# marvinx97/cloud

Measured on AMD Instinct MI355X. Metric: images/sec ResNet-50 via run() at 1/2/4/8 MI355X; run()→first-step latency, higher is better.
Workload: dtype bf16

## Files before the change

### cloud_amd/config.py

```python
from __future__ import annotations

import os
from dataclasses import dataclass


@dataclass(frozen=True)
class Var:
    name: str
    type: type
    default: object
    doc: str
    area: str


_VARS = [
    Var("CLOUD_AMD_JOBS_DIR", str, "./jobs", "where run() stages job directories", "launcher"),
    Var("CLOUD_AMD_HOME", str, "~/.cloud_amd", "per-user state: the job-id index (jobs/<id> -> job directory) that "
        "python -m cloud_amd.jobs uses to find a job from any directory", "launcher"),
    Var("CLOUD_AMD_STAGE_COPY", bool, False, "stage code files by copying too (default: code "
        "hard-linked, every other file copied; a running job then never sees in-place edits of its sources)", "launcher"),
    Var("CLOUD_AMD_CPU_AFFINITY", bool, True, "launcher pins each GPU rank to the cores of its GPU's NUMA node "
        "(KFD io_links + sysfs cpulist), split between the ranks on that node; 0 = leave placement to the OS",
        "launcher"),
    Var("CLOUD_AMD_NUMA_ROOT", str, "/sys/devices/system/node", "sysfs NUMA-node tree read for rank CPU placement "
# ... 49 lines not shown
        "the workgroups (one contiguous sweep); 0 = one contiguous row chunk per workgroup", "ops"),
    Var("CLOUD_AMD_CONV_TALL", bool, True, "<= 64-channel 3x3 convolutions (fwd, stride-1 dgrad): 256 x 64 tiles "
        "with 4 x 1 waves; 0 = 128 x 64 with 2 x 2 waves", "ops"),
    Var("CLOUD_AMD_STEM_LDS", bool, True, "space-to-depth stem convolution forward on the LDS-resident patch + filter "
        "kernel (csrc/include/ca_conv_stem.h); 0 = the implicit-GEMM row-segment loader", "ops"),
    Var("CLOUD_AMD_STEM_TALL", bool, True, "space-to-depth stem convolution on the tall 256 x 64 tiles too (0.88 -> "
        "0.72 ms per call at b1024); 0 = 128 x 64 tiles (A/B runs)", "ops"),
    Var("CLOUD_AMD_STEM_BWD_RECOMPUTE", bool, True, "ResNet stem tail backward: a statistics-only max-pool "
        "backward pass, then the BN-backward apply recomputes the pooled gradient per 2x2 block (the 112x112 "
        "gradient is never written: 3.3 GB fewer per step at b1024).  With the window loads issued ahead of "
        "any branch: 0.65 + 0.90 ms against 1.09 + 0.94 for write-then-apply, +0.8 % end to end "
        "(profiles/r4_s44/); 0 = write g and run the separate apply pass", "ops"),
    Var("CLOUD_AMD_BN_GROUPS_MAX", int, 512, "BatchNorm statistics: most groups of the first-level reduction of the "
        "per-tile partial rows (1..512; ~64 rows per group)", "ops"),
    Var("CLOUD_AMD_GEMM_LIB", str, "never", "plain bf16 GEMMs (bias / accumulate only, no fused epilogue): 'never' "
        "(default: every GEMM on the in-tree kernels, the same engine on every box and rank), 'auto' (diagnostic: "
        "times the in-tree kernel against hipBLASLt once per shape and keeps the faster), 'always' "
        "(ops/raw.py PlainGemmPolicy)", "ops"),
    Var("CLOUD_AMD_GEMM_PRW", bool, True, "forward 1x1 convolutions with N = 256, K = 64 (ResNet layer-1 conv3 "
        "and shortcut): persistent resident-weight core (csrc/include/ca_gemm_prw.h); 0 = the tiled 128 core",
        "ops"),
    Var("CLOUD_AMD_GEMM_PRWN", bool, True, "forward 1x1 convolutions N = 512 / K = 128 and N = 1024 / K = 256 with "
        "BN statistics (ResNet stage-2 / stage-3 conv3): the persistent core with the weight resident in column "
        "chunks (ca_gemm_prw.h); 0 = the tiled 128 core", "ops"),
    Var("CLOUD_AMD_SMALLK_SET", str, "", "bench/smallk_gemm.py shape set ('conv3': the conv3 expansions of "
        "stages 2-4)", "bench"),
    Var("CLOUD_AMD_EPI_PF", bool, True, "GEMM epilogues that read memory or run an activation (BN-statistics "
        "and inference-BN forward 1x1 convs, BERT bias/GELU/GELU'/beta dense layers): 4 staged output rows in flight per trip", "ops"),
    Var("CLOUD_AMD_EPI_PIPE", bool, True, "input-gradient GEMMs / convolutions with the BN-backward statistics "
        "epilogue: the next two output rows' operand loads are in flight under this pair's arithmetic and stores "
        "(ca_mfma_core.h gemm_epilogue); 0 = one pair at a time (A/B runs)", "ops"),
    Var("CLOUD_AMD_ATTN_FUSED_BWD", bool, True,"attention at S = 64 / 128: one workgroup per (batch, head) for "
        "the forward and a single fused backward kernel; 0 keeps the 64-query-block kernels", "ops"),
    Var("CLOUD_AMD_CONV_HALO_WGRAD", bool, True, "the weight gradient of the same 3x3 / 64-channel / width-56 "
        "convolutions on the LDS-resident kernel (ca_conv_halo.h conv3x3_halo_wgrad: 64 x 576 partial in registers, "
        "one fp32 slab per workgroup); 0 = implicit GEMM (A/B)", "ops"),
    Var("CLOUD_AMD_LN_BWD16", bool, False, "LayerNorm backward on 16-wave blocks, one row per wave, the block's "
        "partials summed by a fixed LDS tree (measured 2.8 % slower on BERT beside the weight-gradient side stream; "
        "default: 4-wave blocks walking four rows per wave)", "ops"),
    Var("CLOUD_AMD_GEMM_256X96", bool, True, "forward GEMMs whose 256 x 96 grid fills whole rounds while the 128 x "
        "128 grid leaves a partial one (BERT QKV, M = 8192, N = 2304) run on 256 x 96 tiles; 0 = off (A/B)", "ops"),
    Var("CLOUD_AMD_BN_FIN_RPG", int, 512, "BatchNorm statistics finalize: partial rows per group block (64-512)", "ops"),
    Var("CLOUD_AMD_BN_FIN_MERGED", bool, True, "BatchNorm statistics from many partial rows: group reduction and "
        "per-channel finalize in ONE launch (last block per 64 channels finalizes, agent-scope ticket); 0 = two "
        "launches (A/B runs)", "ops"),
    Var("CLOUD_AMD_CONV_HALO", int, 1, "3x3 / stride-1 / 64-channel convolutions at width 56 (ResNet-50 "
        "stage 1) forward and input gradient on the LDS-resident kernel (ca_conv_halo.h: input patch and all 9 taps "
        "in LDS, persistent grid); 0 = implicit-GEMM tiles, 2 = halo kernel without the software-pipelined "
        "fragment reads (A/B runs)", "ops"),
    Var("CLOUD_AMD_CONV_PATCH", bool, True, "3x3 / stride-1 / pad-1 convolutions with a 64-multiple gathered channel "
        "count, more than 64 output columns and W <= 28 (ResNet-50 stages 2-4), forward and input gradient, on the "
        "patch-fed core (ca_conv_patch.h: the tile's input rows go to LDS once per 64-channel chunk, not once per "
        "tap); 0 = tap-gathered implicit GEMM (A/B runs)", "ops"),
    Var("CLOUD_AMD_CONV_EPI_PF", bool, True, "implicit-GEMM forward convolutions with the BN-statistics epilogue, and "
        "with the inference BN + residual + ReLU epilogue: read 2 staged output rows from LDS before storing", "ops"),
    Var("CLOUD_AMD_INFER_FUSE", bool, True, "ResNet blocks and stem that are not training (eval mode, or a frozen "
        "Keras base) under torch.no_grad(): every BatchNorm (+ residual + ReLU) in the epilogue of its convolution "
        "(ops.conv_bn_act_infer, ca_conv_fwd_bn) and no BN-statistics partials; 0 = the per-layer route "
        "(convolution with statistics, then bn_apply)", "ops"),
    Var("CLOUD_AMD_SHAPE_LOG", str, None, "profiling: append one JSON line per GEMM/convolution launch (kind, M, N, "
        "K, minimum HBM bytes) to this file, for scripts/gemm_roofline.py", "ops"),
    Var("CLOUD_AMD_BN_FOLD", bool, True, "ResNet block backward: the bn3 / bn1 backward apply runs in the operand "
        "fetch of the 1x1 input-gradient GEMM that consumes it (ca_gemm_xa.h) instead of a separate pass", "ops"),
    Var("CLOUD_AMD_BN_FOLD_FWD", bool, True, "ResNet block forward: bn2's apply runs in conv3's operand fetch and "
        "bn3's (+ residual) in the next block's conv1 (ca_gemm_xa.h); the applied tensors are written once, by "
        "those GEMMs", "ops"),
    Var("CLOUD_AMD_BN_FOLD_MAX_N", int, 256, "BN fold sites kept: only GEMMs with K >= 2N and N <= this "
        "(ResNet-50 default: bn3 -> conv3 dgrad and bn3 -> next conv1 at stages 1-3, the stage-3 ones on the two-deep "
        "128 x 256 transform-A tiles, CLOUD_AMD_XA_N256=3: +0.6 / +1.0 % on two boxes, docs/performance.md round 6; "
        "4096 = every stage); the short-K sites (bn2 -> conv3, bn1 -> conv1 dgrad) measured slower than the separate "
        "pass, and stage 4 (N 512) +0.3 % below stages 1-3 only", "ops"),
    Var("CLOUD_AMD_BN_FOLD_WGRAD", bool, True, "bn3 -> conv3 fold at 64 input channels (ResNet stage 1): conv3's weight "
        "gradient runs in the same kernel as its input gradient (ca_gemm_xa.h mfma_gemm_xa_dw), so the BN-backward "
        "output dz3 is never written", "ops"),
    Var("CLOUD_AMD_BN_FOLD_DS", bool, False, "ResNet projection blocks, stages 2-4: the shortcut BN's backward apply "
        "runs in the operand fetch of the sparse strided shortcut input-gradient GEMM (ca_gemm_xa_bwd_strided); A/B",
        "ops"),
    Var("CLOUD_AMD_DS_SPARSE_DGRAD", bool, True, "ResNet projection blocks with a strided 1x1 shortcut: the "
        "shortcut's input gradient is written for its one non-empty output-parity class only, and conv1's input "
        "gradient accumulates into it reading the other pixels as zeros -- no zero-fill of 3/4 of dx and no read "
        "of those zeros", "ops"),
    Var("CLOUD_AMD_BN_FOLD_WGRAD_DS", bool, True, "stage-1 projection shortcut: its BN backward (gated by the block "
        "output's ReLU mask), the shortcut conv's input gradient and its weight gradient in one pass", "ops"),
    Var("CLOUD_AMD_BN_FOLD_WGRAD2", bool, False, "the same one-pass input + weight gradient for stage 2's conv3 "
        "(K = 512 -> N = 128, 8-wave workgroups holding the 512 x 128 dW block)", "ops"),
    Var("CLOUD_AMD_BN_FOLD_WGRAD1", bool, False, "the same one-pass input + weight gradient for stage 1's conv1 with "
        "bn1's backward apply (K = 64 -> N = 256: dz1 never written, four output chunks per tile)", "ops"),
    Var("CLOUD_AMD_XA_N256", int, 3, "transform-A GEMMs (BN folded into a 1x1 conv) with N a multiple of 256: "
        "1 = 128 x 256 tiles on 16-wave workgroups (each A tile transformed once), "
        "3 (and any other value) = 16 waves with two K tiles' operands in flight (coefficients staged in LDS; K <= 2048), "
        "0 = 128 x 128 tiles.  Only the fold sites CLOUD_AMD_BN_FOLD_MAX_N admits reach them (ResNet-50 stage 3 "
        "at the default; measured in docs/performance.md, round 6)", "ops"),
    Var("CLOUD_AMD_XA_WAVES", int, 8,"128 x 128 transform-A GEMMs (BN folded into the 1x1 convs): 8-wave "
        "workgroups (<= 128 registers, two per CU) or 4", "ops"),
    Var("CLOUD_AMD_XA_WAVES_N64", bool, True, "the 128 x 64 transform-A GEMMs (stage 1) on 8-wave workgroups too "
        "(with CLOUD_AMD_XA_WAVES=8)", "ops"),
    Var("CLOUD_AMD_XA_DW_WAVES", int, 4, "stage-1 conv3 fused input+weight gradient: 4-wave workgroups (two per "
        "CU) or 8 (one per CU); 8 selects the one-step form", "ops"),
    Var("CLOUD_AMD_XA_DW_DEPTH", int, 1, "stage-1 fused input+weight gradient (K 256 -> N 64): 0 = one-step form; "
        "1, 2, 4 = deep form (weights resident in LDS, epilogue operands ahead of the next tile's) with that many "
        "source steps in flight per workgroup (1: two workgroups per CU, 2 and 4: one)", "ops"),
    Var("CLOUD_AMD_BN_FOLD_ALL", bool, False, "fold every BN site regardless of CLOUD_AMD_BN_FOLD_MAX_N (tests, A/B)",
        "ops"),
    Var("CLOUD_AMD_MAX_STEPS_IN_FLIGHT", int, 2, "training loops (benches, Keras fit) let the host enqueue at most this "
        "many steps ahead of the GPU (runtime.step_pacer); bounds the memory in flight so the caching allocator "
        "stops requesting segments after warmup; 0 = unbounded", "runtime"),
    Var("CLOUD_AMD_RUN_AHEAD_MS", float, 25.0, "the step pacer deepens its bound (up to 4 steps) so the queued steps "
# ... 143 lines not shown
```

### csrc/bindings.cpp

```cpp
#include <atomic>
#include <mutex>
#include <hip/hip_runtime.h>
#include <pybind11/pybind11.h>
#include <pybind11/stl.h>
#include <stdint.h>

#include <stdexcept>
#include <string>
#include <vector>

namespace py = pybind11;
typedef uint16_t bf16_t;

extern "C" {
int ca_sgd_step(float*, void*, int, float*, bf16_t*, const float*, const float*, long, int, int, hipStream_t);
int ca_adam_step(float*, void*, int, float*, float*, bf16_t*, const float*, const float*, long, int, int, hipStream_t);
int ca_rmsprop_step(float*, void*, int, float*, float*, bf16_t*, const float*, const float*, long, int, hipStream_t);
int ca_sumsq(const void*, int, long, float*, hipStream_t);
int ca_scale(void*, int, long, const float*, hipStream_t);
long ca_bn_workspace_floats(long, int);
int ca_bn_fwd(const bf16_t*, const bf16_t*, bf16_t*, long, int, const float*, const float*, float, float,
              float*, float*, float*, float*, float*, float*, int, uint8_t*, hipStream_t);
int ca_bn_apply(const bf16_t*, const bf16_t*, bf16_t*, long, int, const float*, int, hipStream_t);
int ca_bn_fwd_partials(const bf16_t*, const bf16_t*, bf16_t*, long, int, const float*, int, const float*, const float*,
                       float, float, float*, float*, float*, float*, float*, int, uint8_t*, float*, hipStream_t);
int ca_bn_bwd(const bf16_t*, const bf16_t*, const uint8_t*, const bf16_t*, long, int, const float*, const float*,
              const float*, bf16_t*, bf16_t*, float*, float*, float*, float*, int, hipStream_t);
int ca_bn_bwd_partials(const bf16_t*, const bf16_t*, const uint8_t*, const bf16_t*, long, int, const float*, int,
                       const float*, const float*, const float*, bf16_t*, bf16_t*, float*, float*, float*, float*, int,
                       hipStream_t);
int ca_gemm_bf16_bnstats(int, const bf16_t*, long, const bf16_t*, long, bf16_t*, long, int, int, int, float,
                         const bf16_t*, const uint8_t*, float*, hipStream_t);
long ca_conv_dgrad_stat_tiles(int, int, int, int, int);
long ca_conv_dgrad_stat_rows(int, int, int, int, int, int, int, int, int, int, int, float);
int ca_conv_patch_shape(int, int, int, int, int, int, int, int, int, int, int, int);
long ca_conv_stat_rows(int, int, int, int, int, int, int, int, int, int, int);
int ca_conv_wgrad_splits(int, int, int, int, int, int, int, int, int, int, int, int);
int ca_bn_fwd_partials_ex(const bf16_t*, const bf16_t*, const float*, bf16_t*, long, int, const float*, int,
                          const float*, const float*, float, float, float*, float*, float*, float*, float*, int,
                          uint8_t*, float*, hipStream_t);
int ca_gemm_xa(int, int, const bf16_t*, const bf16_t*, const uint8_t*, const float*, const float*, const float*,
               const float*, bf16_t*, uint8_t*, long, const bf16_t*, long, bf16_t*, long, int, int, int, float, const bf16_t*,
               const uint8_t*, const bf16_t*, const uint8_t*, float*, const bf16_t*, float*, hipStream_t);
int ca_gemm_xa_bwd_strided(const bf16_t*, const bf16_t*, const uint8_t*, const float*, const float*, const float*,
                           bf16_t*, long, const bf16_t*, long, bf16_t*, long, int, int, int, int, int, int, int,
                           hipStream_t);
int ca_gemm_xa_dw(const bf16_t*, const bf16_t*, const uint8_t*, const float*, const float*, const float*, long,
                  const bf16_t*, long, bf16_t*, long, int, int, int, float, const bf16_t*, const uint8_t*,
                  const bf16_t*, const uint8_t*, float*, const bf16_t*, float*, const bf16_t*, long, void*, int, float,
                  float*, int, hipStream_t);
int ca_dgrad_gemm(int, const bf16_t*, long, const bf16_t*, long, bf16_t*, long, int, int, int, float, const bf16_t*,
                  const uint8_t*, const bf16_t*, const uint8_t*, float*, hipStream_t, const bf16_t*, float*, int, int,
                  int);
int ca_conv_dgrad_bnstats(const bf16_t*, const bf16_t*, bf16_t*, int, int, int, int, int, int, int, int, int, int,
                          int, float, const bf16_t*, const uint8_t*, float*, hipStream_t);
int ca_u8_normalize(const uint8_t*, bf16_t*, long, int, const float*, const float*, hipStream_t);
int ca_stem_s2d(const bf16_t*, bf16_t*, int, int, int, int, int, int, int, hipStream_t);
int ca_softmax_xent(const void*, int, const int64_t*, int, int, float, float, float*, float*, void*, hipStream_t);
int ca_softmax_xent_batch(const void*, long, int, const int64_t*, int, int, float, float, float*, float*, void*, float*,
                          float,
                          hipStream_t);
int ca_maxpool_fwd(const bf16_t*, bf16_t*, uint8_t*, int, int, int, int, int, int, int, int, int, hipStream_t);
int ca_maxpool_bwd(const bf16_t*, const uint8_t*, bf16_t*, int, int, int, int, int, int, int, int, int, hipStream_t);
int ca_gap_fwd(const bf16_t*, void*, int, int, int, int, hipStream_t);
int ca_gap_bwd(const void*, int, bf16_t*, int, int, int, hipStream_t);
int ca_gmp_fwd(const bf16_t*, bf16_t*, float*, int, int, int, hipStream_t);
int ca_gmp_bwd(const void*, int, const bf16_t*, const bf16_t*, const float*, bf16_t*, int, int, int, hipStream_t);
int ca_gemm_bf16(int, const bf16_t*, long, const bf16_t*, long, bf16_t*, long, int, int, int, float*, float,
                 hipStream_t);
int ca_gemm_set_core(int);
int ca_gemm_set_xa_n256(int);
int ca_gemm_stat_rows(int, int, int, long, long, long);
int ca_bn_relu_maxpool_s2k3(const bf16_t*, const float*, bf16_t*, uint8_t*, int, int, int, int, int, int, hipStream_t);
int ca_maxpool_bnstats_parts(int, int, int, int);
int ca_maxpool_bwd_s2k3_bnstats(const bf16_t*, const bf16_t*, const uint8_t*, const bf16_t*, bf16_t*, float*, int, int,
                                int, int, int, int, hipStream_t);
int ca_maxpool_bwd_s2k3_bnapply(const bf16_t*, const bf16_t*, const uint8_t*, const bf16_t*, const float*, bf16_t*, int,
                                int, int, int, int, int, hipStream_t);
int ca_conv_fwd_ex(const bf16_t*, const bf16_t*, bf16_t*, int, int, int, int, int, int, int, int, int, int, int,
                   const float*, int, hipStream_t);
int ca_conv_fwd(const bf16_t*, const bf16_t*, bf16_t*, int, int, int, int, int, int, int, int, int, int, int, float*,
                hipStream_t);
int ca_conv_fwd_bn(const bf16_t*, const bf16_t*, bf16_t*, int, int, int, int, int, int, int, int, int, int, int,
                   const float*, const float*, const bf16_t*, int, hipStream_t);
int ca_conv_dgrad(const bf16_t*, const bf16_t*, bf16_t*, int, int, int, int, int, int, int, int, int, int, int, float,
                  hipStream_t, int);
int ca_conv_wgrad(const bf16_t*, const bf16_t*, void*, int, float, int, int, int, int, int, int, int, int, int, int,
                  int, int, float*, hipStream_t);
int ca_splitk_reduce(const float*, int, long, void*, int, float, hipStream_t);
int ca_grad_finalize_multi(const uint64_t*, const float*, int, hipStream_t);
// ... 149 lines not shown
                      u64 mask_out, long lda, u64 B, long ldb, u64 C, long ldc, int M, int N, int K, float beta,
                      u64 res, u64 res_mask, u64 z, u64 mask, u64 stats, u64 z2, u64 stats2, u64 s) {
    check(ca_gemm_xa(layout, mode, P(const bf16_t*, src0), P(const bf16_t*, src1), P(const uint8_t*, mask_in),
                     P(const float*, c0), P(const float*, c1), P(const float*, c2), P(const float*, c3),
                     P(bf16_t*, side),
                     P(uint8_t*, mask_out), lda, P(const bf16_t*, B), ldb, P(bf16_t*, C), ldc, M, N, K, beta,
                     P(const bf16_t*, res), P(const uint8_t*, res_mask), P(const bf16_t*, z), P(const uint8_t*, mask),
                     P(float*, stats), P(const bf16_t*, z2), P(float*, stats2), S(s)),
          "gemm_xa");
  });
  m.def("gemm_xa_bwd_strided", [](u64 src0, u64 src1, u64 mask_in, u64 c0, u64 c1, u64 c2, u64 side, long lda, u64 B,
                                  long ldb, u64 C, long ldc, int M, int N, int K, int Nb, int H, int W, int stride,
                                  u64 s) {
    check(ca_gemm_xa_bwd_strided(P(const bf16_t*, src0), P(const bf16_t*, src1), P(const uint8_t*, mask_in),
                                 P(const float*, c0), P(const float*, c1), P(const float*, c2), P(bf16_t*, side), lda,
                                 P(const bf16_t*, B), ldb, P(bf16_t*, C), ldc, M, N, K, Nb, H, W, stride, S(s)),
          "gemm_xa_bwd_strided");
  });
  m.def("gemm_xa_dw", [](u64 src0, u64 src1, u64 mask_in, u64 c0, u64 c1, u64 c2, long lda, u64 B, long ldb, u64 C,
                         long ldc, int M, int N, int K, float beta, u64 res, u64 res_mask, u64 z, u64 mask, u64 stats,
                         u64 z2, u64 stats2, u64 y, long ldy, u64 dw, int dw_bf16, float dw_beta, u64 ws, int blocks,
                         u64 s) {
    const int g = ca_gemm_xa_dw(P(const bf16_t*, src0), P(const bf16_t*, src1), P(const uint8_t*, mask_in),
                                P(const float*, c0), P(const float*, c1), P(const float*, c2), lda,
                                P(const bf16_t*, B), ldb, P(bf16_t*, C), ldc, M, N, K, beta, P(const bf16_t*, res),
                                P(const uint8_t*, res_mask), P(const bf16_t*, z), P(const uint8_t*, mask),
                                P(float*, stats), P(const bf16_t*, z2), P(float*, stats2), P(const bf16_t*, y), ldy,
                                P(void*, dw), dw_bf16, dw_beta, P(float*, ws), blocks, S(s));
    check(g < 0 ? g : 0, "gemm_xa_dw");
    return g;
  });
  m.def("bn_fwd_partials_ex", [](u64 x, u64 res, u64 res_ss, u64 y, long M, int C, u64 parts, int nparts, u64 gamma,
                                 u64 beta, float eps, float momentum, u64 rm, u64 rv, u64 sm, u64 sr, u64 ss, int relu,
                                 u64 mask, u64 gws, u64 s) {
    check(ca_bn_fwd_partials_ex(P(const bf16_t*, x), P(const bf16_t*, res), P(const float*, res_ss), P(bf16_t*, y), M,
                                C, P(const float*, parts), nparts, P(const float*, gamma), P(const float*, beta), eps,
                                momentum, P(float*, rm), P(float*, rv), P(float*, sm), P(float*, sr), P(float*, ss),
                                relu, P(uint8_t*, mask), P(float*, gws), S(s)),
          "bn_fwd_partials_ex");
  });
  m.def("conv_dgrad_stat_tiles", [](int Nb, int H, int W, int sh, int sw) {
    return ca_conv_dgrad_stat_tiles(Nb, H, W, sh, sw);
  });
  m.def("conv_dgrad_stat_rows", [](int Nb, int H, int W, int Cin, int Cout, int KH, int KW, int sh, int sw, int ph,
                                   int pw, float beta) {
    return ca_conv_dgrad_stat_rows(Nb, H, W, Cin, Cout, KH, KW, sh, sw, ph, pw, beta);
  });
  m.def("conv_stat_rows", [](int Nb, int H, int W, int Cin, int Cout, int KH, int KW, int sh, int sw, int ph,
                             int pw) { return ca_conv_stat_rows(Nb, H, W, Cin, Cout, KH, KW, sh, sw, ph, pw); });
  m.def("conv_patch_shape", [](int Nb, int H, int W, int Cin, int Cout, int KH, int KW, int sh, int sw, int ph,
                               int pw, int dgrad) {
    return ca_conv_patch_shape(Nb, H, W, Cin, Cout, KH, KW, sh, sw, ph, pw, dgrad) != 0;
  });
  m.def("conv_wgrad_splits", [](int Nb, int H, int W, int Cin, int Cout, int KH, int KW, int sh, int sw, int ph,
                                int pw, int fallback) {
    return ca_conv_wgrad_splits(Nb, H, W, Cin, Cout, KH, KW, sh, sw, ph, pw, fallback);
  });
  m.def("conv_dgrad_bnstats", [](u64 dy, u64 w, u64 dx, int Nb, int H, int W, int Cin, int Cout, int KH, int KW,
                                 int sh, int sw, int ph, int pw, float beta, u64 z, u64 mask, u64 stats, u64 s) {
    check(ca_conv_dgrad_bnstats(P(const bf16_t*, dy), P(const bf16_t*, w), P(bf16_t*, dx), Nb, H, W, Cin, Cout, KH, KW,
                                sh, sw, ph, pw, beta, P(const bf16_t*, z), P(const uint8_t*, mask), P(float*, stats),
                                S(s)),
          "conv_dgrad_bnstats");
  });
  m.def("u8_normalize", [](u64 x, u64 y, long n, std::vector<float> mean, std::vector<float> std_, u64 s) {
    if (mean.size() != std_.size() || mean.empty()) throw std::invalid_argument("u8_normalize: mean/std size");
    check(ca_u8_normalize(P(const uint8_t*, x), P(bf16_t*, y), n, (int)mean.size(), mean.data(), std_.data(), S(s)),
          "u8_normalize");
  });
  m.def("stem_s2d", [](u64 x, u64 y, int N, int H, int W, int C, int Hs, int Ws, int pad, u64 s) {
    check(ca_stem_s2d(P(const bf16_t*, x), P(bf16_t*, y), N, H, W, C, Hs, Ws, pad, S(s)), "stem_s2d");
  });
  m.def("softmax_xent", [](u64 z, int zbf, u64 labels, int B, int C, float gscale, float ls, u64 loss, u64 correct,
                           u64 dz, u64 s) {
    check(ca_softmax_xent(P(const void*, z), zbf, P(const int64_t*, labels), B, C, gscale, ls, P(float*, loss),
                          P(float*, correct), P(void*, dz), S(s)), "softmax_xent");
  });
  m.def("softmax_xent_batch", [](u64 z, long ldz, int bf, u64 labels, int B, int C, float gs, float ls, u64 mean, u64 correct,
                                 u64 dz, u64 acc, float acc_w, u64 s) {
    check(ca_softmax_xent_batch(P(const void*, z), ldz, bf, P(const int64_t*, labels), B, C, gs, ls, P(float*, mean),
                                P(float*, correct), P(void*, dz), P(float*, acc), acc_w, S(s)), "softmax_xent_batch");
  });
  m.def("maxpool_fwd", [](u64 x, u64 y, u64 idx, int N, int H, int W, int C, int OH, int OW, int k, int st, int p,
                          u64 s) {
    check(ca_maxpool_fwd(P(const bf16_t*, x), P(bf16_t*, y), P(uint8_t*, idx), N, H, W, C, OH, OW, k, st, p, S(s)),
          "maxpool_fwd");
  });
  m.def("maxpool_bwd", [](u64 dy, u64 idx, u64 dx, int N, int H, int W, int C, int OH, int OW, int k, int st, int p,
                          u64 s) {
    check(ca_maxpool_bwd(P(const bf16_t*, dy), P(const uint8_t*, idx), P(bf16_t*, dx), N, H, W, C, OH, OW, k, st, p,
                         S(s)), "maxpool_bwd");
  });
  m.def("gap_fwd", [](u64 x, u64 y, int ybf, int N, int HW, int C, u64 s) {
    check(ca_gap_fwd(P(const bf16_t*, x), P(void*, y), ybf, N, HW, C, S(s)), "gap_fwd");
  });
  m.def("gemm_bf16", [](int layout, u64 A, long lda, u64 B, long ldb, u64 C, long ldc, int M, int N, int K,
                        u64 stats, float beta, u64 s) {
    check(ca_gemm_bf16(layout, P(const bf16_t*, A), lda, P(const bf16_t*, B), ldb, P(bf16_t*, C), ldc, M, N, K,
                       P(float*, stats), beta, S(s)), "gemm_bf16");
  });
  m.def("conv_fwd", [](u64 x, u64 w, u64 y, int Nb, int H, int W, int Cin, int Cout, int KH, int KW, int sh, int sw,
                       int ph, int pw, u64 stats, u64 s) {
    check(ca_conv_fwd(P(const bf16_t*, x), P(const bf16_t*, w), P(bf16_t*, y), Nb, H, W, Cin, Cout, KH, KW, sh, sw, ph,
                      pw, P(float*, stats), S(s)), "conv_fwd");
  });
  m.def("conv_fwd_bn", [](u64 x, u64 w, u64 y, int Nb, int H, int W, int Cin, int Cout, int KH, int KW, int sh,
// ... 157 lines not shown
```

### csrc/include/ca_mfma_core.h

```cpp
#pragma once
#include "ca_common.h"

namespace ca {

typedef __bf16 bf16x8 __attribute__((ext_vector_type(8)));
typedef short s8v __attribute__((ext_vector_type(8)));
typedef short s4v __attribute__((ext_vector_type(4)));
typedef float f4v __attribute__((ext_vector_type(4)));
typedef __attribute__((address_space(3))) s4v lds_s4v;

typedef unsigned u32x4 __attribute__((ext_vector_type(4)));

constexpr int BK = 64;
constexpr int PAD = 8;

constexpr uint32_t BUF_CAP = 0x7fffffc0u;

__device__ __forceinline__ uint32_t buf_span(long bytes) {
  return bytes <= 0 ? 0u : (bytes >= (long)BUF_CAP ? BUF_CAP : (uint32_t)bytes);
}

enum Epi {
  EPI_BF16 = 0, EPI_F32_PARTIAL = 1, EPI_BF16_BN = 2, EPI_BF16_ST = 3, EPI_BF16_BNR = 4, EPI_BF16_BNR2 = 5,
  EPI_BF16_AFF = 6
// ... 160 lines not shown
}

template <int R, bool KC>
struct TileGeom {
  static constexpr int ROWS = KC ? R : BK;
  static constexpr int COLS = KC ? BK : R;
  static constexpr int LD = COLS + PAD;
  static constexpr int ELEMS = ROWS * LD;
  static constexpr int CHUNKS = ROWS * COLS / 8;
};

template <int R, bool KC>
__device__ __forceinline__ void chunk_coords(int c, int& row, int& col) {
  using G = TileGeom<R, KC>;
  row = c / (G::COLS / 8);
  col = (c % (G::COLS / 8)) * 8;
}

template <int R, bool KC>
__device__ __forceinline__ bf16x8 read_frag(const short* lds, int r0, int k0, int lane) {
  using G = TileGeom<R, KC>;
  if constexpr (KC) {
    s8v v = *reinterpret_cast<const s8v*>(lds + (r0 + (lane & 15)) * G::LD + k0 + 8 * (lane >> 4));
    return __builtin_bit_cast(bf16x8, v);
  } else {
    const int g = lane >> 4, q = (lane & 15) >> 2, p = lane & 3;
    const short* b0 = lds + (k0 + 8 * g + q) * G::LD + r0 + 4 * p;
    s4v lo = __builtin_amdgcn_ds_read_tr16_b64_v4i16((lds_s4v*)(b0));
    s4v hi = __builtin_amdgcn_ds_read_tr16_b64_v4i16((lds_s4v*)(b0 + 4 * G::LD));
    s8v v = {lo[0], lo[1], lo[2], lo[3], hi[0], hi[1], hi[2], hi[3]};
    return __builtin_bit_cast(bf16x8, v);
  }
}

__device__ __forceinline__ int xcd_remap(int bid, int nblk) {
  const int xcd = bid & 7, q = nblk >> 3, r = nblk & 7;
  const int base = xcd < r ? xcd * (q + 1) : r * (q + 1) + (xcd - r) * q;
  return base + (bid >> 3);
}

inline int split_xcd_enabled() {
  static const bool on = env_switch("CLOUD_AMD_SPLIT_XCD", true);
  return on;
}

inline int epi_pipe_enabled() {
  static const bool on = env_switch("CLOUD_AMD_EPI_PIPE", true);
  return on;
}

struct BlkPos {
  int tile, split;
};
__device__ __forceinline__ BlkPos blk_pos(const CoreParams& P) {
  const int nt = gridDim.x;
  if (gridDim.z == 1 || !P.split_xcd) return {xcd_remap(blockIdx.x, nt), (int)blockIdx.z};
  const int lid = xcd_remap(blockIdx.x + nt * blockIdx.z, nt * gridDim.z);
  return {lid % nt, lid / nt};
}
__device__ __forceinline__ int blk_split(const CoreParams& P) { return blk_pos(P).split; }

__device__ __forceinline__ void bar256() {
  __builtin_amdgcn_s_barrier();
  asm volatile("" ::: "memory");
}

template <int N>
__device__ __forceinline__ void vm_wait() {
  asm volatile("s_waitcnt vmcnt(%0)" ::"n"(N) : "memory");
}

__device__ __forceinline__ void lgkm_wait0() { asm volatile("s_waitcnt lgkmcnt(0)" ::: "memory"); }

__device__ __forceinline__ void tile256_coords(int id, int tiles_m, int tiles_n, int& tm, int& tn) {
  constexpr int GM = 4;
  const int per_group = GM * tiles_n;
  const int g = id / per_group;
  const int first_m = g * GM;
  const int rows = (tiles_m - first_m) < GM ? (tiles_m - first_m) : GM;
  const int r = id - g * per_group;
  tm = first_m + r % rows;
  tn = r / rows;
}

__device__ __forceinline__ s8v zero8() { return s8v{0, 0, 0, 0, 0, 0, 0, 0}; }
__device__ __forceinline__ s8v ld16(const bf16_t* p) { return *reinterpret_cast<const s8v*>(p); }


template <int R, int CPT, int NT>
struct DenseKC {
  static constexpr bool KC = true;
  const bf16_t* rowp[CPT];
  int col[CPT];
  bool ok[CPT];
  int K;
  __device__ DenseKC(const CoreParams& P, bool isA, int r0, int tid) {
    const bf16_t* p = isA ? P.A : P.B;
    const long ld = isA ? P.lda : P.ldb;
    const int rlimit = isA ? P.M : P.N;
    K = P.K;
#pragma unroll
    for (int i = 0; i < CPT; ++i) {
      int row, c;
      chunk_coords<R, true>(tid + i * NT, row, c);
      ok[i] = (r0 + row) < rlimit;
      rowp[i] = p + (long)(ok[i] ? r0 + row : 0) * ld;
      col[i] = c;
    }
  }
  __device__ __forceinline__ s8v load(int i, int k0) const {
    const int k = k0 + col[i];
    return (ok[i] && k < K) ? ld16(rowp[i] + k) : zero8();
// ... 749 lines not shown
```

### csrc/kernels/conv.hip

```cpp
#include <stdlib.h>
#include <string.h>

#include "ca_conv_halo.h"
#include "ca_conv_patch.h"
#include "ca_conv_stem.h"
#include "ca_mfma_core.h"

namespace {
using namespace ca;

struct Pix {
  int n, y, x;
};
__device__ __forceinline__ Pix decode(uint32_t m, const FastDiv& dw, const FastDiv& dh) {
  const uint32_t t = fdiv(m, dw);
  const uint32_t x = m - t * dw.d;
  const uint32_t n = fdiv(t, dh);
  return Pix{(int)n, (int)(t - n * dh.d), (int)x};
}

__device__ __forceinline__ void tap_split(int k, int k0, int C, const FastDiv& dc, bool tile_in_tap, int& tap,
                                          int& c) {
  tap = (int)fdiv((uint32_t)(tile_in_tap ? k0 : k), dc);
  c = k - tap * C;
}

template <int R, int CPT, int NT>
struct ConvFwdA {
  static constexpr bool KC = true;
  const CoreParams& P;
  const bf16_t* nbase[CPT];
  int iy0[CPT], ix0[CPT], col[CPT];
  __device__ ConvFwdA(const CoreParams& p, bool, int r0, int tid) : P(p) {
#pragma unroll
    for (int i = 0; i < CPT; ++i) {
      int row, c;
      chunk_coords<R, true>(tid + i * NT, row, c);
      const int m = r0 + row;
      col[i] = c;
      if (m < P.M) {
        const Pix o = decode((uint32_t)m, P.div_ow, P.div_oh);
        nbase[i] = P.A + (long)o.n * P.H * P.W * P.Cin;
        iy0[i] = o.y * P.sh - P.ph;
        ix0[i] = o.x * P.sw - P.pw;
      } else {
        nbase[i] = P.A;
        iy0[i] = -(1 << 29);
        ix0[i] = 0;
      }
    }
  }
  __device__ __forceinline__ s8v load(int i, int k0) const {
    const int k = k0 + col[i];
    if (k >= P.K) return zero8();
    int tap, ci;
    tap_split(k, k0, P.Cin, P.div_cin, P.cin_tile, tap, ci);
// ... 735 lines not shown
          template <int, int, int> class GA, template <int, int, int> class GB, int EPI>
int launch_n64(const CoreParams& p0, hipStream_t s) {
  if (!(tall_tiles() && use_glds())) return launch<128, 64, LA, LB, GA, GB, EPI>(p0, 1, s);
  CoreParams p = p0;
  p.split_xcd = split_xcd_enabled();
  const int tiles = (p.M + 255) / 256;
  if constexpr (EPI == EPI_BF16_ST || EPI == EPI_BF16_AFF) {
    if (conv_epi_pf()) {
      conv_glds_w_kernel<256, 64, 4, 1, GA, GB, EPI, 2><<<dim3(tiles, 1, 1), 256, 0, s>>>(p);
      CA_LAUNCH_CHECK();
      return 0;
    }
  }
  conv_glds_w_kernel<256, 64, 4, 1, GA, GB, EPI><<<dim3(tiles, 1, 1), 256, 0, s>>>(p);
  CA_LAUNCH_CHECK();
  return 0;
}

template <int STATS, bool PIPE>
__global__ void __launch_bounds__(HALO_NT) conv3x3_halo_kernel(HaloParams P) {
  conv3x3_halo<STATS, PIPE>(P);
}

int halo_mode() {
  static int en = -1;
  if (en < 0) {
    const char* e = getenv("CLOUD_AMD_CONV_HALO");
    en = !e ? 1 : (e[0] == '0' ? 0 : (e[0] == '2' ? 2 : 1));
  }
  return en;
}

bool halo_shape(int H, int W, int Cin, int Cout, int KH, int KW, int sh, int sw, int ph, int pw) {
  const int en = halo_mode();
  return en && KH == 3 && KW == 3 && sh == 1 && sw == 1 && ph == 1 && pw == 1 && Cin == HALO_C && Cout == HALO_C &&
         W == 56 && H % HALO_TR == 0 && use_glds();
}

int conv_cus() {
  static int cus = 0;
  if (!cus) {
    int dev = 0;
    hipDeviceProp_t prop;
    cus = (hipGetDevice(&dev) == hipSuccess && hipGetDeviceProperties(&prop, dev) == hipSuccess &&
           prop.multiProcessorCount > 0) ? prop.multiProcessorCount : 256;
  }
  return cus;
}

int halo_grid(int Nb, int H) {
  const int cus = conv_cus();
  const long tiles = (long)Nb * (H / HALO_TR);
  return (int)(tiles < cus ? tiles : cus);
}

__global__ void __launch_bounds__(HWG_NT) conv3x3_halo_wgrad_kernel(HaloWgParams P) { conv3x3_halo_wgrad(P); }

bool halo_wgrad_on() {
  static const bool on = env_switch("CLOUD_AMD_CONV_HALO_WGRAD", true);
  return on;
}

int halo_launch(const bf16_t* x, const bf16_t* w, bf16_t* y, int Nb, int H, int W, float* stats, const bf16_t* bnz,
                const uint8_t* bnmask, int dgrad, hipStream_t s) {
  HaloParams hp{};
  hp.x = x; hp.w = w; hp.y = y; hp.stats = stats; hp.bnz = bnz; hp.bnmask = bnmask;
  hp.N = Nb; hp.H = H; hp.W = W; hp.dgrad = dgrad;
  const int g = halo_grid(Nb, H);
  const bool pipe = halo_mode() != 2;
  const int mode = stats ? (dgrad ? 2 : 1) : 0;
  if (pipe) {
    if (mode == 2) conv3x3_halo_kernel<2, true><<<g, HALO_NT, 0, s>>>(hp);
    else if (mode == 1) conv3x3_halo_kernel<1, true><<<g, HALO_NT, 0, s>>>(hp);
    else conv3x3_halo_kernel<0, true><<<g, HALO_NT, 0, s>>>(hp);
  } else {
    if (mode == 2) conv3x3_halo_kernel<2, false><<<g, HALO_NT, 0, s>>>(hp);
    else if (mode == 1) conv3x3_halo_kernel<1, false><<<g, HALO_NT, 0, s>>>(hp);
    else conv3x3_halo_kernel<0, false><<<g, HALO_NT, 0, s>>>(hp);
  }
  CA_LAUNCH_CHECK();
  return 0;
}

template <bool STATS>
__global__ void __launch_bounds__(STEM_NT) conv_stem_s2d_kernel(StemParams P) {
  conv_stem_s2d<STATS>(P);
}

bool stem_lds_on() {
  static const bool on = env_switch("CLOUD_AMD_STEM_LDS", true);
  return on;
}

bool stem_shape(int H, int W, int Cin, int Cout, int KH, int KW, int sh, int sw, int ph, int pw) {
  return stem_lds_on() && KH == 4 && KW == 4 && sh == 1 && sw == 1 && ph == 0 && pw == 0 && Cin == STEM_CI &&
         Cout == STEM_C && W == STEM_PW && H > 3 && (H - 3) % STEM_TR == 0;
}

int stem_grid(int Nb, int H) {
  const long tiles = (long)Nb * ((H - 3) / STEM_TR);
  const long g = conv_cus();
  return (int)(tiles < g ? tiles : g);
}

int stem_launch(const bf16_t* x, const bf16_t* w, bf16_t* y, int Nb, int H, float* stats, hipStream_t s) {
  StemParams sp{};
// ... 188 lines not shown
        q.dg_kh0 = (py + ph) % sh;
        q.dg_kw0 = (px + pw) % sw;
        q.dg_nh = q.dg_kh0 < KH ? (KH - q.dg_kh0 + sh - 1) / sh : 0;
        q.dg_nw = q.dg_kw0 < KW ? (KW - q.dg_kw0 + sw - 1) / sw : 0;
        q.dg_dy0 = (py + ph - q.dg_kh0) / sh;
        q.dg_dx0 = (px + pw - q.dg_kw0) / sw;
        q.Hq = (H - py + sh - 1) / sh;
        q.Wq = (W - px + sw - 1) / sw;
        if (q.Hq <= 0 || q.Wq <= 0) continue;
        if (skip_empty && q.dg_nh * q.dg_nw == 0) continue;
        q.div_hq = make_fastdiv(q.Hq);
        q.div_wq = make_fastdiv(q.Wq);
        q.div_nw = make_fastdiv(q.dg_nw > 0 ? q.dg_nw : 1);
        q.M = Nb * q.Hq * q.Wq;
        q.K = q.dg_nh * q.dg_nw * Cout;
        q.k_per_split = q.K;
        if (bnz) {
          q.stats = stats + stat_row * 2 * Cin;
          stat_row += (q.M + 127) / 128;
        }
        int rc = bnz ? launch_dgrad_s<EPI_BF16_BN>(q, Cin, s) : launch_dgrad_s<EPI_BF16>(q, Cin, s);
        if (rc) return rc;
      }
    return 0;
  }
  return bnz ? launch_dgrad<EPI_BF16_BN>(p, Cin, s) : launch_dgrad<EPI_BF16>(p, Cin, s);
}

extern "C" {

int ca_conv_dgrad(const bf16_t* dy, const bf16_t* w, bf16_t* dx, int Nb, int H, int W, int Cin, int Cout, int KH,
                  int KW, int sh, int sw, int ph, int pw, float beta, hipStream_t s, int skip_empty) {
  if (skip_empty && (beta != 0.f || (sh == 1 && sw == 1))) return -1;
  return conv_dgrad_impl(dy, w, dx, Nb, H, W, Cin, Cout, KH, KW, sh, sw, ph, pw, beta, nullptr, nullptr, nullptr, s,
                         skip_empty);
}

int ca_conv_dgrad_bnstats(const bf16_t* dy, const bf16_t* w, bf16_t* dx, int Nb, int H, int W, int Cin, int Cout,
                          int KH, int KW, int sh, int sw, int ph, int pw, float beta, const bf16_t* bnz,
                          const uint8_t* bnmask, float* stats, hipStream_t s) {
  if (!bnz || !stats) return -1;
  return conv_dgrad_impl(dy, w, dx, Nb, H, W, Cin, Cout, KH, KW, sh, sw, ph, pw, beta, bnz, bnmask, stats, s);
}

int ca_conv_wgrad(const bf16_t* dy, const bf16_t* x, void* dw, int dw_bf16, float beta, int Nb, int H, int W,
                  int Cin, int Cout, int KH, int KW, int sh, int sw, int ph, int pw, int splits, float* ws,
                  hipStream_t s) {
  if (halo_shape(H, W, Cin, Cout, KH, KW, sh, sw, ph, pw) && halo_wgrad_on() && splits == halo_grid(Nb, H)) {
    HaloWgParams hp{x, dy, ws, Nb, H, W};
    conv3x3_halo_wgrad_kernel<<<splits, HWG_NT, 0, s>>>(hp);
    CA_LAUNCH_CHECK();
    return ca_splitk_reduce(ws, splits, (long)Cout * KH * KW * Cin, dw, dw_bf16, beta, s);
  }
  CoreParams p = conv_params(Nb, H, W, Cin, Cout, KH, KW, sh, sw, ph, pw);
  if (!geom_ok(Cin, Cout, (long)Nb * H * W)) return -1;
  p.A = dy; p.lda = Cout; p.B = x;
  p.M = Cout; p.N = KH * KW * Cin; p.K = Nb * p.OH * p.OW;
  int kps = (p.K / splits + BK - 1) / BK * BK;
  if (kps < BK) kps = BK;
  splits = (p.K + kps - 1) / kps;
  p.k_per_split = kps;
  p.C = ws; p.ldc = p.N; p.split_stride = (long)p.M * p.N;
  int rc;
  if (tapmask_loaders() && (long)p.OH * p.OW >= 2 * BK) {
    if (Cout <= 64)
      rc = (p.N <= 64) ? launch<64, 64, DenseNC, ConvWgradB, GDenseNC, GConvWgradBI, EPI_F32_PARTIAL>(p, splits, s)
                       : launch<64, 128, DenseNC, ConvWgradB, GDenseNC, GConvWgradBI, EPI_F32_PARTIAL>(p, splits, s);
    else
      rc = (p.N <= 64) ? launch<128, 64, DenseNC, ConvWgradB, GDenseNC, GConvWgradBI, EPI_F32_PARTIAL>(p, splits, s)
                       : launch<128, 128, DenseNC, ConvWgradB, GDenseNC, GConvWgradBI, EPI_F32_PARTIAL>(p, splits, s);
    if (rc) return rc;
    return ca_splitk_reduce(ws, splits, (long)p.M * p.N, dw, dw_bf16, beta, s);
  }
  if (tapmask_loaders()) {
    if (Cout <= 64)
      rc = (p.N <= 64) ? launch<64, 64, DenseNC, ConvWgradB, GDenseNC, GConvWgradBT, EPI_F32_PARTIAL>(p, splits, s)
                       : launch<64, 128, DenseNC, ConvWgradB, GDenseNC, GConvWgradBT, EPI_F32_PARTIAL>(p, splits, s);
    else
      rc = (p.N <= 64) ? launch<128, 64, DenseNC, ConvWgradB, GDenseNC, GConvWgradBT, EPI_F32_PARTIAL>(p, splits, s)
                       : launch<128, 128, DenseNC, ConvWgradB, GDenseNC, GConvWgradBT, EPI_F32_PARTIAL>(p, splits, s);
    if (rc) return rc;
    return ca_splitk_reduce(ws, splits, (long)p.M * p.N, dw, dw_bf16, beta, s);
  }
  if (Cout <= 64)
    rc = (p.N <= 64) ? launch<64, 64, DenseNC, ConvWgradB, GDenseNC, GConvWgradB, EPI_F32_PARTIAL>(p, splits, s)
                     : launch<64, 128, DenseNC, ConvWgradB, GDenseNC, GConvWgradB, EPI_F32_PARTIAL>(p, splits, s);
  else
    rc = (p.N <= 64) ? launch<128, 64, DenseNC, ConvWgradB, GDenseNC, GConvWgradB, EPI_F32_PARTIAL>(p, splits, s)
                     : launch<128, 128, DenseNC, ConvWgradB, GDenseNC, GConvWgradB, EPI_F32_PARTIAL>(p, splits, s);
  if (rc) return rc;
  return ca_splitk_reduce(ws, splits, (long)p.M * p.N, dw, dw_bf16, beta, s);
}

int ca_conv_wgrad_splits(int Nb, int H, int W, int Cin, int Cout, int KH, int KW, int sh, int sw, int ph, int pw,
                         int fallback) {
  if (halo_shape(H, W, Cin, Cout, KH, KW, sh, sw, ph, pw) && halo_wgrad_on()) return halo_grid(Nb, H);
  return fallback;
}

int ca_conv_patch_shape(int Nb, int H, int W, int Cin, int Cout, int KH, int KW, int sh, int sw, int ph, int pw,
                        int dgrad) {
  return dgrad ? patch_shape(Nb, H, W, Cout, Cin, KH, KW, sh, sw, ph, pw)
               : patch_shape(Nb, H, W, Cin, Cout, KH, KW, sh, sw, ph, pw);
}

int ca_conv_out_hw(int H, int KH, int sh, int ph) { return (H + 2 * ph - KH) / sh + 1; }

}
```

Baseline: 16620.

## Add patch-fed weight-gradient kernel for 3x3 convolutions at stages 2-4

Adds a new weight-gradient kernel for 3x3 stride-1 convolutions with 128-multiple channel counts and width up to 28. Each workgroup owns all nine taps of a 64x64 channel pair, so each K step loads the input rows into LDS once rather than once per tap. It double-buffers with direct buffer-to-LDS loads and writes split-K partials that the existing reduction sums. The split count is recomputed to suit the new grid. In exchange it carries a large register accumulator (36 MFMA tiles per wave) and pads positions over padded image coordinates, which adds some wasted work.

```diff
diff --git a/cloud_amd/config.py b/cloud_amd/config.py
--- a/cloud_amd/config.py
+++ b/cloud_amd/config.py
@@ -125,7 +125,13 @@
         "count, more than 64 output columns and W <= 28 (ResNet-50 stages 2-4), forward and input gradient, on the "
         "patch-fed core (ca_conv_patch.h: the tile's input rows go to LDS once per 64-channel chunk, not once per "
         "tap); 0 = tap-gathered implicit GEMM (A/B runs)", "ops"),
-    Var("CLOUD_AMD_CONV_EPI_PF", bool, True, "implicit-GEMM forward convolutions with the BN-statistics epilogue, and "
+    Var("CLOUD_AMD_CONV_WGRAD_PATCH", bool, True, "weight gradient of 3x3 / stride-1 / pad-1 convolutions with "
+        "128-multiple channel counts and W <= 28 (ResNet-50 stages 2-4) on the patch-fed weight-gradient core "
+        "(ca_conv_wgrad_patch.h: one workgroup owns the nine taps of a 64 x 64 channel pair, so the input rows go "
+        "to LDS once per K step, not once per tap); 0 = implicit GEMM (A/B runs)", "ops"),
+    Var("CLOUD_AMD_CONV_WGRAD_PATCH_MAXW", int, 28, "widest image the patch-fed weight-gradient core takes (28 = "
+        "stages 2-4, 14 = stages 3-4, 7 = stage 4 only; A/B runs stage by stage)", "ops"),
+    Var("CLOUD_AMD_CONV_EPI_PF", bool, True,"implicit-GEMM forward convolutions with the BN-statistics epilogue, and "
         "with the inference BN + residual + ReLU epilogue: read 2 staged output rows from LDS before storing", "ops"),
     Var("CLOUD_AMD_INFER_FUSE", bool, True, "ResNet blocks and stem that are not training (eval mode, or a frozen "
         "Keras base) under torch.no_grad(): every BatchNorm (+ residual + ReLU) in the epilogue of its convolution "
diff --git a/csrc/bindings.cpp b/csrc/bindings.cpp
--- a/csrc/bindings.cpp
+++ b/csrc/bindings.cpp
@@ -36,6 +36,7 @@
 int ca_conv_patch_shape(int, int, int, int, int, int, int, int, int, int, int, int);
 long ca_conv_stat_rows(int, int, int, int, int, int, int, int, int, int, int);
 int ca_conv_wgrad_splits(int, int, int, int, int, int, int, int, int, int, int, int);
+int ca_conv_wgrad_patch_shape(int, int, int, int, int, int, int, int, int, int, int);
 int ca_bn_fwd_partials_ex(const bf16_t*, const bf16_t*, const float*, bf16_t*, long, int, const float*, int,
                           const float*, const float*, float, float, float*, float*, float*, float*, float*, int,
                           uint8_t*, float*, hipStream_t);
@@ -291,6 +292,10 @@
                                int pw, int dgrad) {
     return ca_conv_patch_shape(Nb, H, W, Cin, Cout, KH, KW, sh, sw, ph, pw, dgrad) != 0;
   });
+  m.def("conv_wgrad_patch_shape", [](int Nb, int H, int W, int Cin, int Cout, int KH, int KW, int sh, int sw, int ph,
+                                     int pw) {
+    return ca_conv_wgrad_patch_shape(Nb, H, W, Cin, Cout, KH, KW, sh, sw, ph, pw) != 0;
+  });
   m.def("conv_wgrad_splits", [](int Nb, int H, int W, int Cin, int Cout, int KH, int KW, int sh, int sw, int ph,
                                 int pw, int fallback) {
     return ca_conv_wgrad_splits(Nb, H, W, Cin, Cout, KH, KW, sh, sw, ph, pw, fallback);
diff --git a/csrc/include/ca_conv_wgrad_patch.h b/csrc/include/ca_conv_wgrad_patch.h
--- /dev/null
+++ b/csrc/include/ca_conv_wgrad_patch.h
@@ -0,0 +1,158 @@
+#pragma once
+#include "ca_mfma_core.h"
+
+namespace ca {
+
+constexpr int WGP_MAXW = 28;
+constexpr int WGP_KS = 64;
+constexpr int wgp_rows(int W) { return (WGP_KS + 2 * (W + 1) + 2 + 31) / 32 * 32; }
+
+struct WgPatchParams {
+  const bf16_t* dy;
+  const bf16_t* x;
+  float* ws;
+  int Nb, H, W, Cin, Cout;
+  int Q;
+  int steps;
+  int nsteps;
+  int split_xcd;
+  FastDiv div_pw, div_h1;
+};
+
+template <int PROWS>
+__device__ __forceinline__ void conv_wgrad_patch(const WgPatchParams& P) {
+  constexpr int NT = 256, R = 64;
+  constexpr int A_ELEMS = WGP_KS * R, X_ELEMS = PROWS * R, STAGE = A_ELEMS + X_ELEMS;
+  constexpr int XI = PROWS / 32;
+  static_assert(PROWS % 32 == 0 && PROWS <= wgp_rows(WGP_MAXW), "patch rows");
+  static_assert(2 * STAGE * 2 <= 48 * 1024, "two workgroups per CU and 64 KiB left for the main stream");
+  __shared__ __attribute__((aligned(16))) short smem[2 * STAGE];
+
+  const int tid = threadIdx.x, lane = tid & 63;
+  const int wave = __builtin_amdgcn_readfirstlane(tid >> 6);
+  const int W = P.W, H = P.H, PW = W + 1;
+  const int need = WGP_KS + 2 * PW + 2;
+  const BlkPos bp = blk_pos(P.split_xcd);
+  const int cchunks = P.Cin / R;
+  const int co0 = (bp.tile / cchunks) * R, ci0 = (bp.tile % cchunks) * R;
+  const int sbeg = bp.split * P.steps;
+  int send = sbeg + P.steps;
+  if (send > P.nsteps) send = P.nsteps;
+
+  const long npix = (long)P.Nb * H * W;
+  const uint32_t a_span = buf_span(npix * P.Cout * 2), x_span = buf_span(npix * P.Cin * 2);
+  const auto ra = __builtin_amdgcn_make_buffer_rsrc(const_cast<bf16_t*>(P.dy), (short)0, (int)a_span, 0x00020000);
+  const auto rx = __builtin_amdgcn_make_buffer_rsrc(const_cast<bf16_t*>(P.x), (short)0, (int)x_span, 0x00020000);
+
+  const int row_t = tid >> 3;
+  const int schunk = ((tid & 7) ^ nc_swz<R>(row_t)) << 3;
+  const uint32_t a_col = (uint32_t)(co0 + schunk) * 2u, x_col = (uint32_t)(ci0 + schunk) * 2u;
+  const uint32_t a_ld = (uint32_t)P.Cout * 2u, x_ld = (uint32_t)P.Cin * 2u;
+  auto pos_off = [&](int q, bool live, uint32_t ld, uint32_t col, uint32_t span) -> uint32_t {
+    const uint32_t uq = (uint32_t)q;
+    const uint32_t t = fdiv(uq, P.div_pw);
+    const uint32_t x = uq - t * (uint32_t)PW;
+    const uint32_t n = fdiv(t, P.div_h1);
+    const uint32_t y = t - n * (uint32_t)(H + 1);
+    const bool ok = live & (uq < (uint32_t)P.Q) & (y < (uint32_t)H) & (x < (uint32_t)W);
+    const uint32_t o = (uq - n * (uint32_t)(H + W + 1) - y) * ld + col;
+    const uint32_t m = 0u - (uint32_t)ok;
+    return (o & m) | (span & ~m);
+  };
+  auto issue = [&](int step, short* stage) {
+    const int q0 = step * WGP_KS;
+#pragma unroll
+    for (int i = 0; i < 2; ++i) {
+      const uint32_t o = pos_off(q0 + row_t + 32 * i, true, a_ld, a_col, a_span);
+      __builtin_amdgcn_raw_ptr_buffer_load_lds(ra, (lds_void*)(stage + (i * NT + wave * 64) * 8), 16, o, 0, 0, 0);
+    }
+#pragma unroll
+    for (int i = 0; i < XI; ++i) {
+      const int r = row_t + 32 * i;
+      const uint32_t o = pos_off(q0 - PW - 1 + r, r < need, x_ld, x_col, x_span);
+      __builtin_amdgcn_raw_ptr_buffer_load_lds(rx, (lds_void*)(stage + A_ELEMS + (i * NT + wave * 64) * 8), 16, o, 0,
+                                               0, 0);
+    }
+  };
+
+  const int g = lane >> 4, fq = (lane & 15) >> 2, fp = lane & 3;
+  auto frag_off = [&](int r0, int k, int (&o)[2]) {
+    const int lc = (r0 >> 3) + (fp >> 1), sub = 4 * (fp & 1);
+    o[0] = k * R + ((lc ^ nc_swz<R>(k)) << 3) + sub;
+    o[1] = (k + 4) * R + ((lc ^ nc_swz<R>(k + 4)) << 3) + sub;
+  };
+  int aoff[4][2], boff[9][2];
+#pragma unroll
+  for (int i = 0; i < 4; ++i) frag_off(i * 16, 8 * g + fq, aoff[i]);
+#pragma unroll
+  for (int j = 0; j < 9; ++j) {
+    const int nf = wave * 9 + j, tap = nf >> 2, cif = nf & 3;
+    const int kh = tap / 3, kw = tap - 3 * kh;
+    frag_off(cif * 16, 8 * g + fq + kh * PW + kw, boff[j]);
+    boff[j][0] += A_ELEMS;
+    boff[j][1] += A_ELEMS;
+  }
+  auto frag = [&](const short* base, const int (&o)[2]) {
+    s4v lo = __builtin_amdgcn_ds_read_tr16_b64_v4i16((lds_s4v*)(base + o[0]));
+    s4v hi = __builtin_amdgcn_ds_read_tr16_b64_v4i16((lds_s4v*)(base + o[1]));
+    s8v v = {lo[0], lo[1], lo[2], lo[3], hi[0], hi[1], hi[2], hi[3]};
+    return __builtin_bit_cast(bf16x8, v);
+  };
+
+  f4v acc[4][9];
+#pragma unroll
+  for (int i = 0; i < 4; ++i)
+#pragma unroll
+    for (int j = 0; j < 9; ++j) acc[i][j] = f4v{0.f, 0.f, 0.f, 0.f};
+
+  auto compute = [&](const short* stage) {
+    bf16x8 af[2][4], bf[2];
+#pragma unroll
+    for (int i = 0; i < 4; ++i) af[0][i] = frag(stage, aoff[i]);
+    bf[0] = frag(stage, boff[0]);
+#pragma unroll
+    for (int t = 0; t < 18; ++t) {
+      const int kk = t / 9, j = t % 9;
+      if (t + 1 < 18) bf[(t + 1) & 1] = frag(stage + ((t + 1) / 9) * 32 * R, boff[(t + 1) % 9]);
+      if (t == 6) {
+#pragma unroll
+        for (int i = 0; i < 4; ++i) af[1][i] = frag(stage + 32 * R, aoff[i]);
+      }
+      __builtin_amdgcn_sched_barrier(0);
+#pragma unroll
+      for (int i = 0; i < 4; ++i)
+        acc[i][j] = __builtin_amdgcn_mfma_f32_16x16x32_bf16(bf[t & 1], af[kk][i], acc[i][j], 0, 0, 0);
+      __builtin_amdgcn_sched_barrier(0);
+    }
+  };
+  auto step = [&](int s, short* __restrict__ cur, short* __restrict__ nxt) {
+    issue(s + 1, nxt);
+    __builtin_amdgcn_sched_barrier(0);
+    compute(cur);
+    asm volatile("s_waitcnt vmcnt(0)" ::: "memory");
+    __syncthreads();
+  };
+
+  issue(sbeg, smem);
+  asm volatile("s_waitcnt vmcnt(0)" ::: "memory");
+  __syncthreads();
+  int s = sbeg;
+#pragma unroll 1
+  for (; s + 1 < send; s += 2) {
+    step(s, smem, smem + STAGE);
+    step(s + 1, smem + STAGE, smem);
+  }
+  if (s < send) compute(smem);
+
+  const long ncols = 9L * P.Cin;
+  float* dst = P.ws + ((long)bp.split * P.Cout + co0 + (lane & 15)) * ncols + ci0 + 4 * g;
+#pragma unroll
+  for (int j = 0; j < 9; ++j) {
+    const int nf = wave * 9 + j, tap = nf >> 2, cif = nf & 3;
+#pragma unroll
+    for (int i = 0; i < 4; ++i)
+      *reinterpret_cast<f4v*>(dst + (long)(16 * i) * ncols + tap * P.Cin + cif * 16) = acc[i][j];
+  }
+}
+
+}
diff --git a/csrc/include/ca_mfma_core.h b/csrc/include/ca_mfma_core.h
--- a/csrc/include/ca_mfma_core.h
+++ b/csrc/include/ca_mfma_core.h
@@ -236,12 +236,13 @@
 struct BlkPos {
   int tile, split;
 };
-__device__ __forceinline__ BlkPos blk_pos(const CoreParams& P) {
+__device__ __forceinline__ BlkPos blk_pos(int split_xcd) {
   const int nt = gridDim.x;
-  if (gridDim.z == 1 || !P.split_xcd) return {xcd_remap(blockIdx.x, nt), (int)blockIdx.z};
+  if (gridDim.z == 1 || !split_xcd) return {xcd_remap(blockIdx.x, nt), (int)blockIdx.z};
   const int lid = xcd_remap(blockIdx.x + nt * blockIdx.z, nt * gridDim.z);
   return {lid % nt, lid / nt};
 }
+__device__ __forceinline__ BlkPos blk_pos(const CoreParams& P) { return blk_pos(P.split_xcd); }
 __device__ __forceinline__ int blk_split(const CoreParams& P) { return blk_pos(P).split; }
 
 __device__ __forceinline__ void bar256() {
diff --git a/csrc/kernels/conv.hip b/csrc/kernels/conv.hip
--- a/csrc/kernels/conv.hip
+++ b/csrc/kernels/conv.hip
@@ -2,6 +2,7 @@
 #include <string.h>
 
 #include "ca_conv_halo.h"
+#include "ca_conv_wgrad_patch.h"
 #include "ca_conv_patch.h"
 #include "ca_conv_stem.h"
 #include "ca_mfma_core.h"
@@ -843,6 +844,70 @@
   const int cus = conv_cus();
   const long tiles = (long)Nb * (H / HALO_TR);
   return (int)(tiles < cus ? tiles : cus);
+}
+
+template <int PROWS>
+__global__ void __launch_bounds__(256, 2) conv_wgrad_patch_kernel(WgPatchParams P) {
+  conv_wgrad_patch<PROWS>(P);
+}
+
+bool conv_wgrad_patch_on() {
+  static const bool on = env_switch("CLOUD_AMD_CONV_WGRAD_PATCH", true);
+  return on;
+}
+
+int conv_wgrad_patch_maxw() {
+  static const int w = [] {
+    const char* e = getenv("CLOUD_AMD_CONV_WGRAD_PATCH_MAXW");
+    const int v = e && e[0] ? atoi(e) : WGP_MAXW;
+    return v < WGP_MAXW ? v : WGP_MAXW;
+  }();
+  return w;
+}
+
+bool conv_wgrad_patch_shape(int Nb, int H, int W, int Cin, int Cout, int KH, int KW, int sh, int sw, int ph, int pw) {
+  if (!(conv_wgrad_patch_on() && KH == 3 && KW == 3 && sh == 1 && sw == 1 && ph == 1 && pw == 1)) return false;
+  if (Nb < 1 || H < 1 || W < 1 || W > conv_wgrad_patch_maxw() || Cin % 128 != 0 || Cout % 128 != 0 || !use_glds())
+    return false;
+  const long npix = (long)Nb * H * W, q = ((long)Nb + 1) * (H + 1) * (W + 1);
+  return npix * Cin * 2 < (long)BUF_CAP && npix * Cout * 2 < (long)BUF_CAP && q + 256 < (1L << 31);
+}
+
+int wgrad_patch_nsteps(int Nb, int H, int W) { return (int)(((long)Nb * (H + 1) * (W + 1) + WGP_KS - 1) / WGP_KS); }
+
+int wgrad_patch_splits(int Nb, int H, int W, int Cin, int Cout, int asked) {
+  const long tiles128 = (long)((Cout + 127) / 128) * ((9 * Cin + 127) / 128);
+  const long pairs = (long)(Cout / 64) * (Cin / 64);
+  const int nsteps = wgrad_patch_nsteps(Nb, H, W);
+  long g = ((asked > 0 ? asked : 1) * tiles128 + pairs - 1) / pairs;
+  const long slots = 2L * conv_cus();
+  if (g * pairs > slots && g * pairs < 2 * slots) g = slots / pairs;
+  if (g < 1) g = 1;
+  if (g > nsteps) g = nsteps;
+  const int per = (int)((nsteps + g - 1) / g);
+  return (nsteps + per - 1) / per;
+}
+
+int launch_wgrad_patch(const bf16_t* dy, const bf16_t* x, float* ws, int Nb, int H, int W, int Cin, int Cout,
+                       int splits, int* eff, hipStream_t s) {
+  WgPatchParams p{};
+  p.dy = dy; p.x = x; p.ws = ws;
+  p.Nb = Nb; p.H = H; p.W = W; p.Cin = Cin; p.Cout = Cout;
+  p.Q = Nb * (H + 1) * (W + 1);
+  p.nsteps = wgrad_patch_nsteps(Nb, H, W);
+  if (splits < 1) splits = 1;
+  if (splits > p.nsteps) splits = p.nsteps;
+  p.steps = (p.nsteps + splits - 1) / splits;
+  splits = (p.nsteps + p.steps - 1) / p.steps;
+  p.split_xcd = split_xcd_enabled();
+  p.div_pw = make_fastdiv(W + 1);
+  p.div_h1 = make_fastdiv(H + 1);
+  const dim3 grid((Cout / 64) * (Cin / 64), 1, splits);
+  if (wgp_rows(W) <= 96) conv_wgrad_patch_kernel<96><<<grid, 256, 0, s>>>(p);
+  else conv_wgrad_patch_kernel<128><<<grid, 256, 0, s>>>(p);
+  CA_LAUNCH_CHECK();
+  *eff = splits;
+  return 0;
 }
 
 __global__ void __launch_bounds__(HWG_NT) conv3x3_halo_wgrad_kernel(HaloWgParams P) { conv3x3_halo_wgrad(P); }
@@ -1137,6 +1202,12 @@
     CA_LAUNCH_CHECK();
     return ca_splitk_reduce(ws, splits, (long)Cout * KH * KW * Cin, dw, dw_bf16, beta, s);
   }
+  if (conv_wgrad_patch_shape(Nb, H, W, Cin, Cout, KH, KW, sh, sw, ph, pw)) {
+    int eff = 0;
+    const int rc = launch_wgrad_patch(dy, x, ws, Nb, H, W, Cin, Cout, splits, &eff, s);
+    if (rc) return rc;
+    return ca_splitk_reduce(ws, eff, (long)Cout * 9 * Cin, dw, dw_bf16, beta, s);
+  }
   CoreParams p = conv_params(Nb, H, W, Cin, Cout, KH, KW, sh, sw, ph, pw);
   if (!geom_ok(Cin, Cout, (long)Nb * H * W)) return -1;
   p.A = dy; p.lda = Cout; p.B = x;
@@ -1180,7 +1251,14 @@
 int ca_conv_wgrad_splits(int Nb, int H, int W, int Cin, int Cout, int KH, int KW, int sh, int sw, int ph, int pw,
                          int fallback) {
   if (halo_shape(H, W, Cin, Cout, KH, KW, sh, sw, ph, pw) && halo_wgrad_on()) return halo_grid(Nb, H);
+  if (conv_wgrad_patch_shape(Nb, H, W, Cin, Cout, KH, KW, sh, sw, ph, pw))
+    return wgrad_patch_splits(Nb, H, W, Cin, Cout, fallback);
   return fallback;
+}
+
+int ca_conv_wgrad_patch_shape(int Nb, int H, int W, int Cin, int Cout, int KH, int KW, int sh, int sw, int ph,
+                              int pw) {
+  return conv_wgrad_patch_shape(Nb, H, W, Cin, Cout, KH, KW, sh, sw, ph, pw);
 }
 
 int ca_conv_patch_shape(int Nb, int H, int W, int Cin, int Cout, int KH, int KW, int sh, int sw, int ph, int pw,
```

Result: no change. 16680, median of 4 (+0.3%).
